# julius-speech/julius

Hardware: AMD Instinct MI355X
Metric: frames_x_states_scored_per_sec (higher is better)
Workload: dtype f32; 1 GPU; C2 = configs[1]: triphone GMM outprob only, S=3000 M=16 D=39, step = 12 launches x 64000 frames; frames_per_launch=64000, parallelism=utterance-sharded x1, kernel=gmm_tile<D=39,FPL=2,NS=16> grid=24000 nsb=16

## Files before the change

### julius_amd/csrc/gmm_api.hip

```cpp
#include "gmm_host.h"

extern "C" {

static int gmm_create_impl(jamd_engine *e, const jamd_gmm_desc *d, int gprune, int gprune_num, jamd_gmm **gp) {
  jamd_gmm **out = gp;
  if (!e || !d || !out) { jamd_set_error("jamd_gmm_create: NULL argument"); return JAMD_EINVAL; }
  *out = nullptr;
  if (d->nstream != 1) {
    jamd_set_error("jamd_gmm_create: nstream=%d; only single-stream models are supported", d->nstream);
    return JAMD_EINVAL;
  }
  if (d->nstate <= 0 || d->veclen <= 0 || d->veclen > 1024 || d->nentry < 0 || d->ndens < 0) {
    jamd_set_error("jamd_gmm_create: bad dimensions S=%d D=%d G=%d E=%d", d->nstate, d->veclen,
                   d->ndens, d->nentry);
    return JAMD_EINVAL;
  }
  if (gprune != JAMD_GPRUNE_NONE && gprune != JAMD_GPRUNE_SAFE && gprune != JAMD_GPRUNE_HEU && gprune != JAMD_GPRUNE_BEAM) {
    jamd_set_error("jamd_gmm_create: unknown gprune method %d", gprune);
    return JAMD_EINVAL;
  }
  const bool history_pruning = gprune == JAMD_GPRUNE_HEU || gprune == JAMD_GPRUNE_BEAM;
  const int requested_gprune = gprune;
  if (history_pruning) gprune = JAMD_GPRUNE_SAFE;
  if (!d->mean || !d->ivar || !d->gconst || !d->st_off || (d->nentry && (!d->ent_dens || !d->ent_logw))) {
    jamd_set_error("jamd_gmm_create: NULL model array");
    return JAMD_EINVAL;
  }
  if (d->st_off[0] != 0 || d->st_off[d->nstate] != d->nentry) {
    jamd_set_error("jamd_gmm_create: st_off must run from 0 to nentry");
    return JAMD_EINVAL;
  }
  JAMD_HIP(hipSetDevice(e->device));
  jamd_gmm *g = new jamd_gmm();
  *gp = g;
  g->eng = e; g->S = d->nstate; g->D = d->veclen; g->E = d->nentry;
  g->gprune = gprune; g->gprune_num = gprune_num;
  const int D = g->D;
  g->rec = ((2 * D + 2) + 3) & ~3;
  const bool have_books = d->nbook > 0 && d->st_book;
  std::vector<int> st_off_plain(g->S + 1, 0), tied;
  std::vector<int> book_first(d->nbook > 0 ? d->nbook : 0, -1);
  for (int s = 0; s < g->S; s++) {
    const int n = d->st_off[s + 1] - d->st_off[s];
    if (n < 0) { jamd_set_error("jamd_gmm_create: st_off not monotone at %d", s); return JAMD_EINVAL; }
    const int b = have_books ? d->st_book[s] : -1;
    if (b >= d->nbook) { jamd_set_error("jamd_gmm_create: codebook id %d out of range", b); return JAMD_EINVAL; }
    if (b >= 0) {
      tied.push_back(s);
      if (book_first[b] < 0) book_first[b] = s;
      else if (n != d->st_off[book_first[b] + 1] - d->st_off[book_first[b]]) {
        jamd_set_error("jamd_gmm_create: states of codebook %d disagree on its size", b); return JAMD_EINVAL;
      }
      st_off_plain[s + 1] = st_off_plain[s];
    } else {
      if (n > g->maxmix) g->maxmix = n;
      st_off_plain[s + 1] = st_off_plain[s] + n;
    }
  }
  g->E_plain = st_off_plain[g->S];
  g->ntied = (int)tied.size();
  if (history_pruning && g->ntied > 0) g->hist_method = requested_gprune;
  g->nbook = g->ntied ? d->nbook : 0;
  if (gprune == JAMD_GPRUNE_SAFE && gprune_num < 1) {
    jamd_set_error("jamd_gmm_create: gprune safe needs gprune_num >= 1"); return JAMD_EINVAL;
  }
  if (gprune == JAMD_GPRUNE_SAFE && gprune_num > 64) {
    jamd_set_error("jamd_gmm_create: gprune_num %d > 64 is not supported on the device", gprune_num);
    return JAMD_EINVAL;
  }
  auto fill_rec = [&](float *r, int dn, float lw) -> bool {
    if (dn >= d->ndens) return false;
    if (dn >= 0) {
      memcpy(r, d->mean + (size_t)dn * D, sizeof(float) * D);
      memcpy(r + D, d->ivar + (size_t)dn * D, sizeof(float) * D);
      r[2 * D] = d->gconst[dn];
      if (r[2 * D] != r[2 * D]) g->has_null = true;
    } else {
      r[2 * D] = __builtin_nanf("");
      g->has_null = true;
    }
    r[2 * D + 1] = lw;
    return true;
  };
  std::vector<float> rec((size_t)g->E_plain * g->rec, 0.0f);
  for (int s = 0; s < g->S; s++) {
    if (have_books && d->st_book[s] >= 0) continue;
    for (int k = 0; k < d->st_off[s + 1] - d->st_off[s]; k++) {
      const int en = d->st_off[s] + k;
      if (!fill_rec(rec.data() + (size_t)(st_off_plain[s] + k) * g->rec, d->ent_dens[en], d->ent_logw[en])) {
        jamd_set_error("jamd_gmm_create: density index %d out of range", d->ent_dens[en]); return JAMD_EINVAL;
      }
    }
  }
  JAMD_HIP(hipMalloc(&g->d_rec, sizeof(float) * (rec.size() ? rec.size() : 4)));
  JAMD_HIP(hipMemcpy(g->d_rec, rec.data(), sizeof(float) * rec.size(), hipMemcpyHostToDevice));
  JAMD_HIP(hipMalloc(&g->d_st_off, sizeof(int) * (g->S + 1)));
  JAMD_HIP(hipMemcpy(g->d_st_off, d->st_off, sizeof(int) * (g->S + 1), hipMemcpyHostToDevice));
  JAMD_HIP(hipMalloc(&g->d_st_off_plain, sizeof(int) * (g->S + 1)));
  JAMD_HIP(hipMemcpy(g->d_st_off_plain, st_off_plain.data(), sizeof(int) * (g->S + 1), hipMemcpyHostToDevice));
  if (g->ntied) {
    std::vector<int> book_off(g->nbook + 1, 0);
    for (int b = 0; b < g->nbook; b++) {
      const int n = book_first[b] >= 0 ? d->st_off[book_first[b] + 1] - d->st_off[book_first[b]] : 0;
      book_off[b + 1] = book_off[b] + n;
      if (n > g->maxbook) g->maxbook = n;
    }
    std::vector<float> brec((size_t)book_off[g->nbook] * g->rec, 0.0f);
    for (int b = 0; b < g->nbook; b++) {
      if (book_first[b] < 0) continue;
      for (int k = 0; k < book_off[b + 1] - book_off[b]; k++) {
        if (!fill_rec(brec.data() + (size_t)(book_off[b] + k) * g->rec,
                      d->ent_dens[d->st_off[book_first[b]] + k], 0.0f)) {
          jamd_set_error("jamd_gmm_create: codebook density index out of range"); return JAMD_EINVAL;
        }
      }
    }
    g->tm_cap = (gprune == JAMD_GPRUNE_NONE) ? g->maxbook : (gprune_num < g->maxbook ? gprune_num : g->maxbook);
    JAMD_HIP(hipMalloc(&g->d_book_rec, sizeof(float) * (brec.size() ? brec.size() : 4)));
    JAMD_HIP(hipMemcpy(g->d_book_rec, brec.data(), sizeof(float) * brec.size(), hipMemcpyHostToDevice));
    g->h_book_off = book_off;
    JAMD_HIP(hipMalloc(&g->d_book_off, sizeof(int) * (g->nbook + 1)));
    JAMD_HIP(hipMemcpy(g->d_book_off, book_off.data(), sizeof(int) * (g->nbook + 1), hipMemcpyHostToDevice));
    JAMD_HIP(hipMalloc(&g->d_st_book, sizeof(int) * g->S));
    JAMD_HIP(hipMemcpy(g->d_st_book, d->st_book, sizeof(int) * g->S, hipMemcpyHostToDevice));
    JAMD_HIP(hipMalloc(&g->d_ent_logw, sizeof(float) * (g->E ? g->E : 1)));
    JAMD_HIP(hipMemcpy(g->d_ent_logw, d->ent_logw, sizeof(float) * g->E, hipMemcpyHostToDevice));
    JAMD_HIP(hipMalloc(&g->d_tied_states, sizeof(int) * g->ntied));
    JAMD_HIP(hipMemcpy(g->d_tied_states, tied.data(), sizeof(int) * g->ntied, hipMemcpyHostToDevice));
  }
  return JAMD_OK;
}


int jamd_gmm_create(jamd_engine *e, const jamd_gmm_desc *d, int gprune, int gprune_num,
                    jamd_gmm **out) {
  if (!e || !d || !out) { jamd_set_error("jamd_gmm_create: NULL argument"); return JAMD_EINVAL; }
  *out = nullptr;
  jamd_gmm *g = nullptr;
  const int rc = gmm_create_impl(e, d, gprune, gprune_num, &g);
  if (rc != JAMD_OK) { if (g) jamd_gmm_destroy(g); return rc; }
  *out = g;
  return JAMD_OK;
}

void jamd_gmm_destroy(jamd_gmm *g) {
  if (!g) return;
  (void)hipSetDevice(g->eng->device);
  void *ptrs[] = { g->d_rec, g->d_cur_utt_off, g->d_st_off, g->d_st_off_plain, g->d_tied_states, g->d_st_book, g->d_book_off, g->d_book_rec,
                   g->d_ent_logw, g->d_frames, g->d_out, g->d_tm_score, g->d_tm_id, g->d_tm_num, g->d_narrow };
  for (void *p : ptrs) if (p) (void)hipFree(p);
  if (g->h_utt_off) (void)hipHostFree(g->h_utt_off);
  if (g->ev_utt_off) (void)hipEventDestroy(g->ev_utt_off);
  delete g;
}

int jamd_gmm_nstate(const jamd_gmm *g) { return g ? g->S : -1; }
int jamd_gmm_veclen(const jamd_gmm *g) { return g ? g->D : -1; }
const char *jamd_gmm_last_kernel(const jamd_gmm *g) { return g ? g->last_kernel : ""; }

int jamd_gmm_nentry(const jamd_gmm *g) {
  if (!g) return 0;
  if (g->ntied == 0) return g->E;
  if (g->ntied == g->S && !g->h_book_off.empty()) return g->h_book_off[g->nbook];
  return 0;
}

int jamd_gmm_book_offsets(const jamd_gmm *g, int *off, int cap) {
  if (!g || !off || g->ntied != g->S || (int)g->h_book_off.size() != g->nbook + 1 || cap < g->nbook + 1) {
    jamd_set_error("jamd_gmm_book_offsets: not an all-tied-mixture model, or buffer too small"); return JAMD_EINVAL;
  }
  memcpy(off, g->h_book_off.data(), sizeof(int) * (size_t)(g->nbook + 1));
  return JAMD_OK;
}

int jamd_gmm_dens_dev(jamd_gmm *g, const float *dev_frames, int T, float *dev_out, void *stream) {
  if (!g || !dev_frames || !dev_out || T < 0) { jamd_set_error("jamd_gmm_dens_dev: bad argument"); return JAMD_EINVAL; }
  const int E = jamd_gmm_nentry(g);
  if (E <= 0) {
    jamd_set_error("jamd_gmm_dens_dev: models mixing plain and tied-mixture states have no single column order");
    return JAMD_EINVAL;
  }
  if (T == 0) return JAMD_OK;
  JAMD_HIP(hipSetDevice(g->eng->device));
  hipStream_t st = jamd_stream(g->eng, stream);
  const int rc = jamd_gmm_launch_dens(g, g->ntied ? g->d_book_rec : g->d_rec, E, dev_frames, T, dev_out, st);
  if (rc != JAMD_OK) return rc;
  hipError_t le = hipGetLastError();
  if (le != hipSuccess) { jamd_set_error("jamd_gmm_dens_dev: launch failed: %s", hipGetErrorString(le)); return JAMD_ELAUNCH; }
  return JAMD_OK;
}

int jamd_gmm_dens_host(jamd_gmm *g, const float *host_frames, int T, float *host_out) {
  if (!g || !host_frames || !host_out || T < 0) { jamd_set_error("jamd_gmm_dens_host: bad argument"); return JAMD_EINVAL; }
  if (T == 0) return JAMD_OK;
  JAMD_HIP(hipSetDevice(g->eng->device));
  float *d_fr = nullptr, *d_out = nullptr;
  int rc = JAMD_OK;
  hipStream_t st = g->eng->stream;
  const int E = jamd_gmm_nentry(g);
  if (E <= 0) { jamd_set_error("jamd_gmm_dens_host: no single column order for this model"); return JAMD_EINVAL; }
  if (hipMalloc(&d_fr, sizeof(float) * (size_t)T * g->D) != hipSuccess ||
      hipMalloc(&d_out, sizeof(float) * (size_t)T * E) != hipSuccess) {
    jamd_set_error("jamd_gmm_dens_host: out of device memory"); rc = JAMD_ENOMEM;
  }
  if (rc == JAMD_OK && hipMemcpyAsync(d_fr, host_frames, sizeof(float) * (size_t)T * g->D, hipMemcpyHostToDevice, st) != hipSuccess) rc = JAMD_ENODEV;
  if (rc == JAMD_OK) rc = jamd_gmm_dens_dev(g, d_fr, T, d_out, st);
  if (rc == JAMD_OK && (hipMemcpyAsync(host_out, d_out, sizeof(float) * (size_t)T * E, hipMemcpyDeviceToHost, st) != hipSuccess ||
                        hipStreamSynchronize(st) != hipSuccess)) { jamd_set_error("jamd_gmm_dens_host: copy failed"); rc = JAMD_ELAUNCH; }
  if (d_fr) (void)hipFree(d_fr);
  if (d_out) (void)hipFree(d_out);
  return rc;
}

static int set_utterances(jamd_gmm *g, const int *utt_off, int nutt, hipStream_t st) {
  if (g->hist_method == 0) return JAMD_OK;
  int rc;
  if ((rc = jamd_grow(&g->d_cur_utt_off, &g->utt_off_bytes, sizeof(int) * ((size_t)nutt + 1))) != JAMD_OK) return rc;
  if (g->ev_utt_off) JAMD_HIP(hipEventSynchronize(g->ev_utt_off));
  else JAMD_HIP(hipEventCreateWithFlags(&g->ev_utt_off, hipEventDisableTiming));
  if ((size_t)(nutt + 1) > g->h_utt_off_cap) {
    if (g->h_utt_off) JAMD_HIP(hipHostFree(g->h_utt_off));
    g->h_utt_off = nullptr; g->h_utt_off_cap = 0;
    const size_t cap = (size_t)nutt + 1 < 1024 ? 1024 : (size_t)nutt + 1;
    JAMD_HIP(hipHostMalloc((void **)&g->h_utt_off, sizeof(int) * cap, hipHostMallocDefault));
    g->h_utt_off_cap = cap;
  }
  memcpy(g->h_utt_off, utt_off, sizeof(int) * ((size_t)nutt + 1));
  JAMD_HIP(hipMemcpyAsync(g->d_cur_utt_off, g->h_utt_off, sizeof(int) * ((size_t)nutt + 1), hipMemcpyHostToDevice, st));
  JAMD_HIP(hipEventRecord(g->ev_utt_off, st));
  g->cur_nutt = nutt;
  return JAMD_OK;
}

int jamd_gmm_outprob_dev(jamd_gmm *g, const float *dev_frames, int T, float *dev_out, void *stream) {
  const int off[2] = {0, T};
  if (T < 0) { jamd_set_error("jamd_gmm_outprob_dev: bad argument"); return JAMD_EINVAL; }
  return jamd_gmm_outprob_utts_dev(g, dev_frames, off, 1, dev_out, stream);
}

int jamd_gmm_outprob_utts_dev(jamd_gmm *g, const float *dev_frames, const int *utt_off, int nutt, float *dev_out, void *stream) {
  if (!g || !dev_frames || !dev_out || !utt_off || nutt < 1 || utt_off[0] != 0) {
    jamd_set_error("jamd_gmm_outprob_utts_dev: bad argument");
    return JAMD_EINVAL;
  }
  for (int u = 0; u < nutt; u++)
    if (utt_off[u + 1] < utt_off[u]) { jamd_set_error("jamd_gmm_outprob_utts_dev: utt_off must be non-decreasing"); return JAMD_EINVAL; }
  const int T = utt_off[nutt];
  if (T == 0) return JAMD_OK;
  JAMD_HIP(hipSetDevice(g->eng->device));
  hipStream_t st = jamd_stream(g->eng, stream);
  int rc = JAMD_OK;
  if ((rc = set_utterances(g, utt_off, nutt, st)) != JAMD_OK) return rc;
  if (g->E_plain == 0 && g->ntied == g->S) {
  } else if (g->gprune == JAMD_GPRUNE_SAFE) {
    rc = jamd_gmm_launch_safe(g, dev_frames, T, dev_out, st);
  } else {
    rc = jamd_gmm_launch_plain(g, dev_frames, T, dev_out, st);
  }
  if (rc != JAMD_OK) return rc;
  if (g->ntied) {
    const size_t n = (size_t)T * g->nbook * g->tm_cap;
    if ((rc = jamd_grow(&g->d_tm_score, &g->tm_cap_bytes, sizeof(float) * n)) != JAMD_OK) return rc;
    if ((rc = jamd_grow(&g->d_tm_id, &g->tm_id_bytes, sizeof(int) * n)) != JAMD_OK) return rc;
    if ((rc = jamd_grow(&g->d_tm_num, &g->tm_num_bytes, sizeof(int) * (size_t)T * g->nbook)) != JAMD_OK) return rc;
    if ((rc = jamd_gmm_launch_tmix(g, dev_frames, T, dev_out, g->d_tm_score, g->d_tm_id, g->d_tm_num, st)) != JAMD_OK) return rc;
  }
  hipError_t le = hipGetLastError();
  if (le != hipSuccess) {
    jamd_set_error("jamd_gmm_outprob_dev: launch failed: %s", hipGetErrorString(le));
    return JAMD_ELAUNCH;
  }
  return JAMD_OK;
}

int jamd_gmm_outprob_host(jamd_gmm *g, const float *host_frames, int T, float *host_out) {
  if (!g || !host_frames || !host_out || T < 0) {
    jamd_set_error("jamd_gmm_outprob_host: bad argument");
    return JAMD_EINVAL;
  }
  if (T == 0) return JAMD_OK;
  JAMD_HIP(hipSetDevice(g->eng->device));
  int rc;
  if ((rc = jamd_grow(&g->d_frames, &g->frames_cap, sizeof(float) * (size_t)T * g->D)) != JAMD_OK) return rc;
  if ((rc = jamd_grow(&g->d_out, &g->out_cap, sizeof(float) * (size_t)T * g->S)) != JAMD_OK) return rc;
  hipStream_t st = g->eng->stream;
  JAMD_HIP(hipMemcpyAsync(g->d_frames, host_frames, sizeof(float) * (size_t)T * g->D,
                          hipMemcpyHostToDevice, st));
  if ((rc = jamd_gmm_outprob_dev(g, g->d_frames, T, g->d_out, st)) != JAMD_OK) return rc;
  JAMD_HIP(hipMemcpyAsync(host_out, g->d_out, sizeof(float) * (size_t)T * g->S,
                          hipMemcpyDeviceToHost, st));
  hipError_t se = hipStreamSynchronize(st);
  if (se != hipSuccess) {
    jamd_set_error("jamd_gmm_outprob_host: execution failed: %s", hipGetErrorString(se));
    return JAMD_ELAUNCH;
  }
  return JAMD_OK;
}

int jamd_gmm_tmix_cap(const jamd_gmm *g) { return g ? g->tm_cap : -1; }
int jamd_gmm_nbook(const jamd_gmm *g) { return g ? g->nbook : -1; }

int jamd_gmm_tmix_cache_dev(jamd_gmm *g, const float *dev_frames, int T, float *dev_score,
                            int *dev_id, int *dev_num, void *stream) {
  if (!g || !dev_frames || !dev_score || !dev_id || !dev_num || T < 0) {
    jamd_set_error("jamd_gmm_tmix_cache_dev: bad argument");
    return JAMD_EINVAL;
  }
  if (!g->ntied) { jamd_set_error("jamd_gmm_tmix_cache_dev: model has no tied-mixture states"); return JAMD_ESTATE; }
  if (T == 0) return JAMD_OK;
  JAMD_HIP(hipSetDevice(g->eng->device));
  const int off[2] = {0, T};
  int rc = set_utterances(g, off, 1, jamd_stream(g->eng, stream));
  if (rc == JAMD_OK) rc = jamd_gmm_launch_tmix(g, dev_frames, T, nullptr, dev_score, dev_id, dev_num, jamd_stream(g->eng, stream));
  if (rc != JAMD_OK) return rc;
  hipError_t le = hipGetLastError();
  if (le != hipSuccess) {
    jamd_set_error("jamd_gmm_tmix_cache_dev: launch failed: %s", hipGetErrorString(le));
    return JAMD_ELAUNCH;
  }
  return JAMD_OK;
}

}
```

### julius_amd/csrc/gmm_host.h

```cpp
#pragma once
#include <vector>

#include "jamd_internal.h"

struct jamd_gmm {
  jamd_engine *eng = nullptr;
  int S = 0, D = 0, E = 0, nbook = 0;
  int gprune = 0, gprune_num = 0;
  int rec = 0;
  int maxmix = 0;
  float *d_rec = nullptr;
  int *d_st_off = nullptr;
  int *d_st_off_plain = nullptr;
  int E_plain = 0;
  int *d_st_book = nullptr;
  int *d_book_off = nullptr;
  std::vector<int> h_book_off;
  float *d_book_rec = nullptr;
  float *d_ent_logw = nullptr;
  int *d_tied_states = nullptr;
  int ntied = 0;
  int maxbook = 0;
  int tm_cap = 0;
  bool has_null = false;
  int hist_method = 0;
  int *d_cur_utt_off = nullptr;
  int cur_nutt = 0; size_t utt_off_bytes = 0;
  float *d_frames = nullptr; size_t frames_cap = 0;
  float *d_out = nullptr; size_t out_cap = 0;
  float *d_tm_score = nullptr; int *d_tm_id = nullptr; int *d_tm_num = nullptr;
  float *d_narrow = nullptr; size_t narrow_cap = 0;
  size_t tm_cap_bytes = 0, tm_id_bytes = 0, tm_num_bytes = 0;
  char last_kernel[64] = {0};
  int *h_utt_off = nullptr; size_t h_utt_off_cap = 0; hipEvent_t ev_utt_off = nullptr;
};

#define JAMD_GMM_LOCAL __attribute__((visibility("hidden")))

JAMD_GMM_LOCAL int jamd_gmm_launch_plain(jamd_gmm *g, const float *frames, int T, float *out, hipStream_t st);
JAMD_GMM_LOCAL int jamd_gmm_launch_dens(jamd_gmm *g, const float *rec, int E, const float *frames, int T, float *out,
                                        hipStream_t st);

int jamd_gmm_launch_safe(jamd_gmm *g, const float *frames, int T, float *out, hipStream_t st);
int jamd_gmm_launch_tmix(jamd_gmm *g, const float *frames, int T, float *out, float *c_score,
                         int *c_id, int *c_num, hipStream_t st);
```

### julius_amd/csrc/gmm_outprob.hip

```cpp
#include "gmm_dev.h"
#include "gmm_host.h"

namespace {
using namespace jamd;

constexpr int kWaves = 4;

template <int D, int FPL, int NS, bool HAS_NULL>
__global__ void __launch_bounds__(64 * kWaves)
gmm_tile_kernel(const float *__restrict__ rec, const int *__restrict__ st_off,
                const float *__restrict__ frames, const float *__restrict__ tbl,
                float *__restrict__ out, int T, int S, int nsb, int nfb, int nstb,
                float addmin_f) {
  static_assert(FPL % 2 == 0, "frames are processed as packed pairs");
  constexpr int REC = ((2 * D + 2) + 3) & ~3;
  constexpr int FPW = 64 * FPL;
  constexpr int NP = FPL / 2;
  __shared__ float tile[kWaves][FPW][NS + 1];

  int fb, sb;
  if (!decode_block(nfb, nstb, fb, sb)) return;
  const int lane = threadIdx.x & 63;
  const int wave = threadIdx.x >> 6;
  const int t0 = (fb * kWaves + wave) * FPW;
  if (t0 >= T) return;

  f2 v[NP][D];
#pragma unroll
  for (int p = 0; p < NP; p++) load_frames<D>(v[p], nullptr, frames, t0 + p * 128, T, D, lane);

#if defined(__HIP_DEVICE_COMPILE__) && !defined(__GFX9__)
#error "gmm_tile: the raw buffer descriptor below is the gfx9 (CDNA) format; this library is written for gfx950 only"
#endif
  const __amdgpu_buffer_rsrc_t tbl_rsrc = __builtin_amdgcn_make_buffer_rsrc((void *)tbl, 0, 4 * (JAMD_TBLSIZE + 1), 0x00020000);
  const int s_begin = sb * nsb;
  const int s_end = min(S, s_begin + nsb);
  for (int sg = s_begin; sg < s_end; sg += NS) {
    const int ns = min(NS, s_end - sg);
    for (int si = 0; si < ns; si++) {
      const int e0 = st_off[sg + si], e1 = st_off[sg + si + 1];
      f2 y2[NP], tv2[NP];
#pragma unroll
      for (int p = 0; p < NP; p++) { y2[p] = f2{JAMD_LOG_ZERO, JAMD_LOG_ZERO}; tv2[p] = f2{0.0f, 0.0f}; }
      for (int e = e1 - 1; e >= e0; e--) {
        const float *__restrict__ r = rec + (size_t)e * REC;
        const float gc = r[2 * D], lw = r[2 * D + 1];
        f2 acc[NP];
#pragma unroll
        for (int p = 0; p < NP; p++) acc[p] = f2{gc, gc};
#pragma unroll
        for (int d = 0; d < D; d++) {
          const float mu = r[d], iv = r[D + d];
          const f2 mu2 = {mu, mu}, iv2 = {iv, iv};
#pragma unroll
          for (int p = 0; p < NP; p++) {
            f2 x = v[p][d] - mu2;
            x = x * x;
            x = x * iv2;
            acc[p] = acc[p] + x;
          }
        }
        const bool nulld = HAS_NULL && (gc != gc);
        const float naddmin = -addmin_f;
#pragma unroll
        for (int p = 0; p < NP; p++) {
          f2 s2 = acc[p] * f2{-0.5f, -0.5f};
          if (nulld) s2 = f2{JAMD_LOG_ZERO, JAMD_LOG_ZERO};
          s2 = s2 + f2{lw, lw};
          __builtin_amdgcn_sched_barrier(0);
          const f2 yy = y2[p] + tv2[p];
          const f2 hi = {__builtin_fmaxf(s2.x, yy.x), __builtin_fmaxf(s2.y, yy.y)};
          const f2 df = s2 - yy;
          const float a0 = __builtin_fabsf(df.x), a1 = __builtin_fabsf(df.y);
          unsigned o0 = ((unsigned)((double)a0 * JAMD_TMAG + 0.5)) << 2, o1 = ((unsigned)((double)a1 * JAMD_TMAG + 0.5)) << 2;
          o0 = (a0 <= naddmin) ? o0 : 4u * (unsigned)JAMD_TBLSIZE;
          o1 = (a1 <= naddmin) ? o1 : 4u * (unsigned)JAMD_TBLSIZE;
          tv2[p] = f2{__builtin_bit_cast(float, __builtin_amdgcn_raw_buffer_load_b32(tbl_rsrc, (int)o0, 0, 0)),
                      __builtin_bit_cast(float, __builtin_amdgcn_raw_buffer_load_b32(tbl_rsrc, (int)o1, 0, 0))};
          y2[p] = hi;
        }
      }
#pragma unroll
      for (int k = 0; k < FPL; k++) {
        const f2 fin = y2[k / 2] + tv2[k / 2];
        tile[wave][k * 64 + lane][si] = finish_state((k & 1) ? fin.y : fin.x);
      }
    }
    wave_sync();
    constexpr int RPI = 64 / NS;
    const int col = lane % NS, rsub = lane / NS;
#pragma unroll 4
    for (int it = 0; it < FPW / RPI; it++) {
      const int rr = it * RPI + rsub;
      const int t = t0 + rr;
      if (t < T && col < ns) out[(size_t)t * S + sg + col] = tile[wave][rr][col];
    }
    wave_release();
  }
}

template <int FPL, int NS>
__global__ void __launch_bounds__(64 * kWaves)
gmm_tile_generic_kernel(const float *__restrict__ rec, const int *__restrict__ st_off,
                        const float *__restrict__ frames, const float *__restrict__ tbl,
                        float *__restrict__ out, int T, int S, int D, int REC, int nsb, int nfb,
                        int nstb, float addmin_f) {
  static_assert(FPL == 2, "load_frames / gauss_pair hold one packed pair of frames per lane");
  constexpr int FPW = 64 * FPL;
  __shared__ float tile[kWaves][FPW][NS + 1];
  extern __shared__ __align__(16) float dyn[];

  int fb, sb;
  if (!decode_block(nfb, nstb, fb, sb)) return;
  const int lane = threadIdx.x & 63;
  const int wave = threadIdx.x >> 6;
  const int t0 = (fb * kWaves + wave) * FPW;
  if (t0 >= T) return;
  float *vt = dyn + (size_t)wave * D * FPW;
  load_frames<0>(nullptr, vt, frames, t0, T, D, lane);

  const int s_begin = sb * nsb;
  const int s_end = min(S, s_begin + nsb);
  for (int sg = s_begin; sg < s_end; sg += NS) {
    const int ns = min(NS, s_end - sg);
    for (int si = 0; si < ns; si++) {
      const int e0 = st_off[sg + si], e1 = st_off[sg + si + 1];
      float y0 = JAMD_LOG_ZERO, y1 = JAMD_LOG_ZERO;
      for (int e = e1 - 1; e >= e0; e--) {
        const float *__restrict__ r = rec + (size_t)e * REC;
        const float lw = r[2 * D + 1];
        const f2 g = gauss_pair<0>(nullptr, vt, lane, D, r);
        y0 = addlog_step(y0, g.x + lw, tbl, addmin_f);
        y1 = addlog_step(y1, g.y + lw, tbl, addmin_f);
      }
      tile[wave][lane][si] = finish_state(y0);
      tile[wave][64 + lane][si] = finish_state(y1);
    }
    store_tile<NS, FPW>(tile[wave], out, t0, T, S, sg, ns, lane);
  }
}

template <int D, int FPL, int NS>
int launch_tile(jamd_gmm *g, const float *frames, int T, float *out, hipStream_t st) {
  constexpr int FPB = kWaves * 64 * FPL;
  const int nfb = (T + FPB - 1) / FPB;
  const int nsb = NS;
  const int nstb = (g->S + nsb - 1) / nsb;
  const int grid = xcd_grid(nstb, nfb);
  if (g->has_null)
    hipLaunchKernelGGL((gmm_tile_kernel<D, FPL, NS, true>), dim3(grid), dim3(64 * kWaves), 0, st,
                       g->d_rec, g->d_st_off_plain, frames, g->eng->d_addlog, out, T, g->S, nsb, nfb,
                       nstb, g->eng->addmin_f);
  else
    hipLaunchKernelGGL((gmm_tile_kernel<D, FPL, NS, false>), dim3(grid), dim3(64 * kWaves), 0, st,
                       g->d_rec, g->d_st_off_plain, frames, g->eng->d_addlog, out, T, g->S, nsb, nfb,
                       nstb, g->eng->addmin_f);
  snprintf(g->last_kernel, sizeof(g->last_kernel), "gmm_tile<D=%d,FPL=%d,NS=%d> grid=%d nsb=%d", D, FPL, NS, grid, nsb);
  return JAMD_OK;
}

template <int FPL, int NS>
int launch_tile_generic(jamd_gmm *g, const float *frames, int T, float *out, hipStream_t st) {
  constexpr int FPB = kWaves * 64 * FPL;
  const int nfb = (T + FPB - 1) / FPB;
  const int nsb = NS;
  const int nstb = (g->S + nsb - 1) / nsb;
  const int grid = xcd_grid(nstb, nfb);
  const size_t dyn = sizeof(float) * kWaves * g->D * 64 * FPL;
  const int rc = jamd_reserve_dyn_lds((const void *)gmm_tile_generic_kernel<FPL, NS>, dyn, "GMM outprob");
  if (rc != JAMD_OK) return rc;
  hipLaunchKernelGGL((gmm_tile_generic_kernel<FPL, NS>), dim3(grid), dim3(64 * kWaves), dyn, st,
                     g->d_rec, g->d_st_off_plain, frames, g->eng->d_addlog, out, T, g->S, g->D, g->rec,
                     nsb, nfb, nstb, g->eng->addmin_f);
  snprintf(g->last_kernel, sizeof(g->last_kernel), "gmm_tile_generic<FPL=%d,NS=%d> D=%d grid=%d",
           FPL, NS, g->D, grid);
  return JAMD_OK;
}

constexpr int kNarrowT = 256;
constexpr int kNarrowFB = 8;
template <int D, bool HAS_NULL>
__global__ void __launch_bounds__(64)
gmm_narrow_dens_kernel(const float *__restrict__ rec, const float *__restrict__ frames, float *__restrict__ dens, int T, int E,
                       int nfb, int neb) {
  constexpr int REC = (2 * D + 2 + 3) & ~3;
  int fbk, ebk;
  if (!decode_block(nfb, neb, fbk, ebk)) return;
  const int e = ebk * 64 + threadIdx.x;
  const float4 *__restrict__ r4 = reinterpret_cast<const float4 *>(rec + (size_t)(e < E ? e : E - 1) * REC);
  float r[REC];
#pragma unroll
  for (int q = 0; q < REC / 4; q++) { const float4 v = r4[q]; r[4 * q] = v.x; r[4 * q + 1] = v.y; r[4 * q + 2] = v.z; r[4 * q + 3] = v.w; }
  const float gc = r[2 * D], lw = r[2 * D + 1];
  const bool nulld = HAS_NULL && (gc != gc);
  const int t_end = min(T, (fbk + 1) * kNarrowFB);
  for (int t = fbk * kNarrowFB; t < t_end; t += 2) {
    const float *__restrict__ fa = frames + (size_t)t * D;
    const float *__restrict__ fb = frames + (size_t)(t + 1 < T ? t + 1 : t) * D;
    f2 acc = {gc, gc};
#pragma unroll
    for (int d = 0; d < D; d++) {
      f2 x = f2{fa[d], fb[d]} - f2{r[d], r[d]};
      x = x * x;
      x = x * f2{r[D + d], r[D + d]};
      acc = acc + x;
    }
    f2 s2 = acc * f2{-0.5f, -0.5f};
    if (nulld) s2 = f2{JAMD_LOG_ZERO, JAMD_LOG_ZERO};
    s2 = s2 + f2{lw, lw};
    if (e < E) {
      dens[(size_t)t * E + e] = s2.x;
      if (t + 1 < T) dens[(size_t)(t + 1) * E + e] = s2.y;
    }
  }
}

__global__ void __launch_bounds__(256)
gmm_narrow_lse_kernel(const float *__restrict__ dens, const int *__restrict__ st_off, const float *__restrict__ tbl,
                      float *__restrict__ out, int T, int S, int E, float addmin_f) {
  const int i = blockIdx.x * 256 + threadIdx.x;
  if (i >= T * S) return;
  const int t = i / S, s = i - t * S;
  const int e0 = st_off[s], e1 = st_off[s + 1];
  const float *__restrict__ dr = dens + (size_t)t * E;
  float y = JAMD_LOG_ZERO;
  int e = e1 - 1;
  for (; e - 7 >= e0; e -= 8) {
    float v[8];
#pragma unroll
    for (int q = 0; q < 8; q++) v[q] = dr[e - q];
#pragma unroll
    for (int q = 0; q < 8; q++) y = addlog_step(y, v[q], tbl, addmin_f);
  }
  for (; e >= e0; e--) y = addlog_step(y, dr[e], tbl, addmin_f);
  out[(size_t)t * S + s] = finish_state(y);
}

template <int D>
int launch_narrow(jamd_gmm *g, const float *frames, int T, float *out, hipStream_t st) {
  const int E = g->E_plain;
  int rc = jamd_grow(&g->d_narrow, &g->narrow_cap, sizeof(float) * (size_t)kNarrowT * (size_t)E);
  if (rc != JAMD_OK) return rc;
  const int grid = (E + 63) / 64;
  const int nfb = (T + kNarrowFB - 1) / kNarrowFB;
  const dim3 gr(xcd_grid(grid, nfb));
  if (g->has_null) hipLaunchKernelGGL((gmm_narrow_dens_kernel<D, true>), gr, dim3(64), 0, st, g->d_rec, frames, g->d_narrow, T, E, nfb, grid);
  else hipLaunchKernelGGL((gmm_narrow_dens_kernel<D, false>), gr, dim3(64), 0, st, g->d_rec, frames, g->d_narrow, T, E, nfb, grid);
  hipLaunchKernelGGL(gmm_narrow_lse_kernel, dim3((T * g->S + 255) / 256), dim3(256), 0, st, g->d_narrow, g->d_st_off_plain,
                     g->eng->d_addlog, out, T, g->S, E, g->eng->addmin_f);
  snprintf(g->last_kernel, sizeof(g->last_kernel), "gmm_narrow<D=%d> grid=%d + lse", D, grid);
  return JAMD_OK;
}

constexpr int kDensChunk = 1024;
__global__ void __launch_bounds__(64)
gmm_dens_kernel(const float *__restrict__ rec, const float *__restrict__ frames, float *__restrict__ out,
                int T, int E, int D, int REC) {
  extern __shared__ float xs[];
  float (*tile)[17] = reinterpret_cast<float (*)[17]>(xs + (size_t)D * 64);
  const int lane = threadIdx.x;
  const int t0 = blockIdx.x * 64, e_begin = blockIdx.y * kDensChunk;
  const int e_end = min(E, e_begin + kDensChunk);
  {
    int t = t0 + lane; if (t > T - 1) t = T - 1;
    const float *f = frames + (size_t)t * D;
    for (int d = 0; d < D; d++) xs[d * 64 + lane] = f[d];
  }
  wave_sync();
  for (int e0 = e_begin; e0 < e_end; e0 += 16) {
    const int ne = min(16, e_end - e0);
    for (int g = 0; g < ne; g++) {
      const float *__restrict__ r = rec + (size_t)(e0 + g) * REC;
      const float gc = r[2 * D];
      float acc = gc;
      for (int d = 0; d < D; d++) {
        float x = xs[d * 64 + lane] - r[d];
        x = x * x;
        x = x * r[D + d];
        acc = acc + x;
      }
      float sc = acc * -0.5f;
      if (gc != gc) sc = JAMD_LOG_ZERO;
      tile[lane][g] = sc;
    }
    wave_sync();
    const int col = lane & 15, rsub = lane >> 4;
    for (int it = 0; it < 16; it++) {
      const int rr = it * 4 + rsub, t = t0 + rr;
      if (t < T && col < ne) out[(size_t)t * E + e0 + col] = tile[rr][col];
    }
    wave_release();
  }
}

}


int jamd_gmm_launch_plain(jamd_gmm *g, const float *frames, int T, float *out, hipStream_t st) {
  const bool narrow = T <= kNarrowT && g->E_plain > 0;
  return dispatch_veclen(g->D, [&](auto dt) {
    constexpr int D = decltype(dt)::value;
    if constexpr (D == 0) return launch_tile_generic<2, 16>(g, frames, T, out, st);
    else return narrow ? launch_narrow<D>(g, frames, T, out, st) : launch_tile<D, 2, 16>(g, frames, T, out, st);
  });
}

int jamd_gmm_launch_dens(jamd_gmm *g, const float *rec, int E, const float *frames, int T, float *out, hipStream_t st) {
  const size_t lds = sizeof(float) * ((size_t)g->D * 64 + 64 * 17);
  if (lds > 64 * 1024) { jamd_set_error("jamd_gmm_dens_dev: vector length %d too large", g->D); return JAMD_EINVAL; }
  hipLaunchKernelGGL(gmm_dens_kernel, dim3((T + 63) / 64, (E + kDensChunk - 1) / kDensChunk), dim3(64), lds, st,
                     rec, frames, out, T, E, g->D, g->rec);
  return JAMD_OK;
}
```

Before: 19.08 billion frame*states/s.

## Add D=39 ring kernel with scalar prefetch of Gaussian records

Adds a D=39 specialised kernel that reads each Gaussian's mean/ivar/gconst/weight from a host-reordered 80-float record through explicit s_load_dwordx16 scalar loads. Three 16-float register chunks are rotated so the next mixture's record is prefetched while the current one is computed, and the next state's first record is fetched ahead of time as well. The addlog table lookup goes through a buffer resource. This aims to hide scalar-memory latency behind the per-mixture ALU work. In exchange it relies on inline asm and sched_barriers, uses more SGPRs, needs an extra device copy of the parameters, and the hand-written waitcnt placement is fragile.

```diff
diff --git a/julius_amd/csrc/gmm_api.hip b/julius_amd/csrc/gmm_api.hip
--- a/julius_amd/csrc/gmm_api.hip
+++ b/julius_amd/csrc/gmm_api.hip
@@ -94,6 +94,20 @@
   }
   JAMD_HIP(hipMalloc(&g->d_rec, sizeof(float) * (rec.size() ? rec.size() : 4)));
   JAMD_HIP(hipMemcpy(g->d_rec, rec.data(), sizeof(float) * rec.size(), hipMemcpyHostToDevice));
+  if (D == 39) {
+    constexpr int kRing = 80;
+    std::vector<float> ring((size_t)g->E_plain * kRing, 0.0f);
+    for (int en = 0; en < g->E_plain; en++) {
+      const float *r = rec.data() + (size_t)en * g->rec;
+      float *q = ring.data() + (size_t)en * kRing;
+      q[0] = r[2 * D]; q[1] = r[2 * D + 1];
+      for (int k = 0; k < 7; k++) { q[2 + k] = r[k]; q[9 + k] = r[D + k]; }
+      for (int c = 1; c < 5; c++)
+        for (int k = 0; k < 8; k++) { q[16 * c + k] = r[8 * c - 1 + k]; q[16 * c + 8 + k] = r[D + 8 * c - 1 + k]; }
+    }
+    JAMD_HIP(hipMalloc(&g->d_rec_ring, sizeof(float) * (ring.size() ? ring.size() : 4)));
+    JAMD_HIP(hipMemcpy(g->d_rec_ring, ring.data(), sizeof(float) * ring.size(), hipMemcpyHostToDevice));
+  }
   JAMD_HIP(hipMalloc(&g->d_st_off, sizeof(int) * (g->S + 1)));
   JAMD_HIP(hipMemcpy(g->d_st_off, d->st_off, sizeof(int) * (g->S + 1), hipMemcpyHostToDevice));
   JAMD_HIP(hipMalloc(&g->d_st_off_plain, sizeof(int) * (g->S + 1)));
@@ -146,7 +160,7 @@
 void jamd_gmm_destroy(jamd_gmm *g) {
   if (!g) return;
   (void)hipSetDevice(g->eng->device);
-  void *ptrs[] = { g->d_rec, g->d_cur_utt_off, g->d_st_off, g->d_st_off_plain, g->d_tied_states, g->d_st_book, g->d_book_off, g->d_book_rec,
+  void *ptrs[] = { g->d_rec, g->d_rec_ring, g->d_cur_utt_off, g->d_st_off, g->d_st_off_plain, g->d_tied_states, g->d_st_book, g->d_book_off, g->d_book_rec,
                    g->d_ent_logw, g->d_frames, g->d_out, g->d_tm_score, g->d_tm_id, g->d_tm_num, g->d_narrow };
   for (void *p : ptrs) if (p) (void)hipFree(p);
   if (g->h_utt_off) (void)hipHostFree(g->h_utt_off);
diff --git a/julius_amd/csrc/gmm_host.h b/julius_amd/csrc/gmm_host.h
--- a/julius_amd/csrc/gmm_host.h
+++ b/julius_amd/csrc/gmm_host.h
@@ -10,6 +10,7 @@
   int rec = 0;
   int maxmix = 0;
   float *d_rec = nullptr;
+  float *d_rec_ring = nullptr;
   int *d_st_off = nullptr;
   int *d_st_off_plain = nullptr;
   int E_plain = 0;
diff --git a/julius_amd/csrc/gmm_outprob.hip b/julius_amd/csrc/gmm_outprob.hip
--- a/julius_amd/csrc/gmm_outprob.hip
+++ b/julius_amd/csrc/gmm_outprob.hip
@@ -99,6 +99,117 @@
   }
 }
 
+typedef float f16v __attribute__((ext_vector_type(16)));
+constexpr int kRingRec = 80;
+
+template <int BYTE_OFF>
+__device__ __forceinline__ void ring_load(f16v &home, const float *chunks) {
+  __builtin_amdgcn_sched_barrier(0);
+  asm volatile("s_load_dwordx16 %0, %1, %2" : "=s"(home) : "s"(chunks), "i"(BYTE_OFF));
+  __builtin_amdgcn_sched_barrier(0);
+}
+__device__ __forceinline__ void ring_wait(f16v &h0, f16v &h1, f16v &h2) {
+  __builtin_amdgcn_sched_barrier(0);
+  asm volatile("s_waitcnt lgkmcnt(0)" : "+s"(h0), "+s"(h1), "+s"(h2));
+  __builtin_amdgcn_sched_barrier(0);
+}
+template <int N, int MU0, int IV0>
+__device__ __forceinline__ void ring_chunk(f2 &acc, const f2 *v, const f16v &h) {
+  f2 x[N], q[N], w[N];
+#pragma unroll
+  for (int i = 0; i < N + 3; i++) {
+    if (i < N) { const float mu = h[MU0 + i]; x[i] = v[i] - f2{mu, mu}; }
+    if (i >= 1 && i - 1 < N) q[i - 1] = x[i - 1] * x[i - 1];
+    if (i >= 2 && i - 2 < N) { const float iv = h[IV0 + i - 2]; w[i - 2] = q[i - 2] * f2{iv, iv}; }
+    if (i >= 3) acc = acc + w[i - 3];
+    __builtin_amdgcn_sched_barrier(0);
+  }
+}
+
+template <int NS, bool HAS_NULL>
+__global__ void __launch_bounds__(64 * kWaves)
+gmm_tile_ring_kernel(const float *__restrict__ ring, const int *__restrict__ st_off,
+                     const float *__restrict__ frames, const float *__restrict__ tbl,
+                     float *__restrict__ out, int T, int S, int nsb, int nfb, int nstb,
+                     float addmin_f) {
+  constexpr int D = 39, FPL = 2;
+  constexpr int FPW = 64 * FPL;
+  __shared__ float tile[kWaves][FPW][NS + 1];
+
+  int fb, sb;
+  if (!decode_block(nfb, nstb, fb, sb)) return;
+  const int lane = threadIdx.x & 63;
+  const int wave = threadIdx.x >> 6;
+  const int t0 = (fb * kWaves + wave) * FPW;
+  if (t0 >= T) return;
+
+  f2 v[D];
+  load_frames<D>(v, nullptr, frames, t0, T, D, lane);
+
+  const __amdgpu_buffer_rsrc_t tbl_rsrc = __builtin_amdgcn_make_buffer_rsrc((void *)tbl, 0, 4 * (JAMD_TBLSIZE + 1), 0x00020000);
+  const float naddmin = -addmin_f;
+  const int s_begin = sb * nsb;
+  const int s_end = min(S, s_begin + nsb);
+  f16v h0, h1, h2;
+  int held = -1;
+  for (int sg = s_begin; sg < s_end; sg += NS) {
+    const int ns = min(NS, s_end - sg);
+    for (int si = 0; si < ns; si++) {
+      const int s = sg + si;
+      const int e0 = st_off[s], e1 = st_off[s + 1];
+      const int e_over = (s + 1 < s_end ? st_off[s + 2] : e1) - 1;
+      f2 y2 = {JAMD_LOG_ZERO, JAMD_LOG_ZERO}, tv2 = {0.0f, 0.0f};
+      if (e1 > e0 && held != e1 - 1) {
+        const float *r = ring + (size_t)(e1 - 1) * kRingRec;
+        ring_load<0>(h0, r);
+        ring_load<64>(h1, r);
+        ring_load<128>(h2, r);
+        ring_wait(h0, h1, h2);
+      }
+      for (int e = e1 - 1; e >= e0; e--) {
+        const float *r = ring + (size_t)e * kRingRec;
+        const float *rn = ring + (size_t)(e > e0 ? e - 1 : e_over) * kRingRec;
+        const float gc = h0[0], lw = h0[1];
+        const bool nulld = HAS_NULL && (gc != gc);
+        f2 acc = {gc, gc};
+        ring_chunk<7, 2, 9>(acc, v, h0);
+        ring_load<192>(h0, r);
+        ring_chunk<8, 0, 8>(acc, v + 7, h1);
+        ring_load<256>(h1, r);
+        ring_chunk<8, 0, 8>(acc, v + 15, h2);
+        ring_wait(h0, h1, h2);
+        ring_chunk<8, 0, 8>(acc, v + 23, h0);
+        ring_load<0>(h0, rn);
+        ring_load<128>(h2, rn);
+        ring_chunk<8, 0, 8>(acc, v + 31, h1);
+        ring_load<64>(h1, rn);
+        {
+          f2 s2 = acc * f2{-0.5f, -0.5f};
+          if (nulld) s2 = f2{JAMD_LOG_ZERO, JAMD_LOG_ZERO};
+          s2 = s2 + f2{lw, lw};
+          __builtin_amdgcn_sched_barrier(0);
+          const f2 yy = y2 + tv2;
+          const f2 hi = {__builtin_fmaxf(s2.x, yy.x), __builtin_fmaxf(s2.y, yy.y)};
+          const f2 df = s2 - yy;
+          const float a0 = __builtin_fabsf(df.x), a1 = __builtin_fabsf(df.y);
+          unsigned o0 = ((unsigned)((double)a0 * JAMD_TMAG + 0.5)) << 2, o1 = ((unsigned)((double)a1 * JAMD_TMAG + 0.5)) << 2;
+          o0 = (a0 <= naddmin) ? o0 : 4u * (unsigned)JAMD_TBLSIZE;
+          o1 = (a1 <= naddmin) ? o1 : 4u * (unsigned)JAMD_TBLSIZE;
+          tv2 = f2{__builtin_bit_cast(float, __builtin_amdgcn_raw_buffer_load_b32(tbl_rsrc, (int)o0, 0, 0)),
+                   __builtin_bit_cast(float, __builtin_amdgcn_raw_buffer_load_b32(tbl_rsrc, (int)o1, 0, 0))};
+          y2 = hi;
+        }
+        ring_wait(h0, h1, h2);
+      }
+      if (e1 > e0) held = e_over;
+      const f2 fin = y2 + tv2;
+      tile[wave][lane][si] = finish_state(fin.x);
+      tile[wave][64 + lane][si] = finish_state(fin.y);
+    }
+    store_tile<NS, FPW>(tile[wave], out, t0, T, S, sg, ns, lane);
+  }
+}
+
 template <int FPL, int NS>
 __global__ void __launch_bounds__(64 * kWaves)
 gmm_tile_generic_kernel(const float *__restrict__ rec, const int *__restrict__ st_off,
@@ -147,15 +258,27 @@
   const int nsb = NS;
   const int nstb = (g->S + nsb - 1) / nsb;
   const int grid = xcd_grid(nstb, nfb);
-  if (g->has_null)
-    hipLaunchKernelGGL((gmm_tile_kernel<D, FPL, NS, true>), dim3(grid), dim3(64 * kWaves), 0, st,
-                       g->d_rec, g->d_st_off_plain, frames, g->eng->d_addlog, out, T, g->S, nsb, nfb,
-                       nstb, g->eng->addmin_f);
-  else
-    hipLaunchKernelGGL((gmm_tile_kernel<D, FPL, NS, false>), dim3(grid), dim3(64 * kWaves), 0, st,
-                       g->d_rec, g->d_st_off_plain, frames, g->eng->d_addlog, out, T, g->S, nsb, nfb,
-                       nstb, g->eng->addmin_f);
-  snprintf(g->last_kernel, sizeof(g->last_kernel), "gmm_tile<D=%d,FPL=%d,NS=%d> grid=%d nsb=%d", D, FPL, NS, grid, nsb);
+  if constexpr (D == 39 && FPL == 2) {
+    if (g->has_null)
+      hipLaunchKernelGGL((gmm_tile_ring_kernel<NS, true>), dim3(grid), dim3(64 * kWaves), 0, st,
+                         g->d_rec_ring, g->d_st_off_plain, frames, g->eng->d_addlog, out, T, g->S, nsb, nfb,
+                         nstb, g->eng->addmin_f);
+    else
+      hipLaunchKernelGGL((gmm_tile_ring_kernel<NS, false>), dim3(grid), dim3(64 * kWaves), 0, st,
+                         g->d_rec_ring, g->d_st_off_plain, frames, g->eng->d_addlog, out, T, g->S, nsb, nfb,
+                         nstb, g->eng->addmin_f);
+    snprintf(g->last_kernel, sizeof(g->last_kernel), "gmm_tile<D=%d,FPL=%d,NS=%d,ring> grid=%d nsb=%d", D, FPL, NS, grid, nsb);
+  } else {
+    if (g->has_null)
+      hipLaunchKernelGGL((gmm_tile_kernel<D, FPL, NS, true>), dim3(grid), dim3(64 * kWaves), 0, st,
+                         g->d_rec, g->d_st_off_plain, frames, g->eng->d_addlog, out, T, g->S, nsb, nfb,
+                         nstb, g->eng->addmin_f);
+    else
+      hipLaunchKernelGGL((gmm_tile_kernel<D, FPL, NS, false>), dim3(grid), dim3(64 * kWaves), 0, st,
+                         g->d_rec, g->d_st_off_plain, frames, g->eng->d_addlog, out, T, g->S, nsb, nfb,
+                         nstb, g->eng->addmin_f);
+    snprintf(g->last_kernel, sizeof(g->last_kernel), "gmm_tile<D=%d,FPL=%d,NS=%d> grid=%d nsb=%d", D, FPL, NS, grid, nsb);
+  }
   return JAMD_OK;
 }
 
```

Measured after the change: 19.48 billion frame*states/s (median of 6 runs). +2.1%, better.
